# x-y20/jittor-dcn

Hardware: NVIDIA B200
Metric: DeformConv2d fwd+bwd images/sec (higher is better)
Workload: dtype f32

## Files before the change

jittor_dcn_b200/csrc/dcn_umma_bwd_data.cu:

```cuda
#include <cstdlib>
#include <cstring>
#include <type_traits>

#include "dcn_umma.h"
#include "dcn_umma_common.cuh"

namespace dcn {

using namespace ptx;

namespace bd {

constexpr int kScatWarps = 16;
constexpr int kMmaWarp = kScatWarps, kLoadWarp = kScatWarps + 1;
constexpr int kFirstPlanWarp = kScatWarps + 2;
__host__ __device__ constexpr int threads_of(int pw) { return (kFirstPlanWarp + pw) * 32; }
constexpr int kPlanPerThread = 8;
__host__ __device__ constexpr int plan_max_of(int pw) { return pw * 32 * kPlanPerThread; }
constexpr uint32_t kGImg = 128 * 64 * 2;

struct __align__(16) ScatEntry {
  uint32_t base;
  float fx, fy;
  uint32_t gidx;
};
constexpr uint32_t kDeadEntry = 0xffffffffu;

struct Params {
  Geo g;
  Tiling t;
  const void* xt;
  float* gxt;
  const float* off;
  const void* gout;
  const uint8_t* wtiles;
  const uint8_t* gtiles;
  float* gb_fused;
  int row_v;
  float* goff;
  float scale_iy, scale_ix;
  int Gt, Rt, chunks, num_inst;
  int num_tiles;
  FastDiv divR, divChunks;
  int pix_blocks;
  int ix_delta;
  int ncols;
  int cblocks;
  int OB;
  int plan_cap;
  int fuse_w;
  int o_halves;
  int o_cols;
  float* gw;
  int nslices, nchunks, cb_per_slice;
  int g_imgs;
  int g_nbuf;
  uint32_t g_img;
  uint32_t w_stage;
  uint32_t tmem_cols;
  int w_resident;
  int w_ring;
};

struct PlanWork {
  float ox, oy;
  int h, w, n, chan_base, valid;
  uint32_t gidx;
  float mk;
};

template <int VARIANT, bool PLAIN = false, bool MOD = false>
__device__ __forceinline__ void plan_prepare(const Params& P, int tile, int cb, int e, PlanWork& pw,
                                             const float* __restrict__ mask = nullptr) {
  const Geo& g = P.g;
  pw.valid = 0;
  pw.ox = pw.oy = 0.f;
  pw.h = pw.w = pw.n = pw.chan_base = 0;
  pw.gidx = kDeadEntry;
  uint32_t p, n, h, w;
  int b;
  if (VARIANT == DCN_VARIANT_TORCH) {
    const int il = e >> (P.ncols == 128 ? 7 : 6), cc = e & (P.ncols - 1), j = cb * P.ncols + cc;
    const TileRowInfo ri = decode_inst(P, tile * P.Rt + il);
    if (!ri.valid || j >= g.K) return;
    uint32_t cbase, q;
    P.t.divP.divmod((uint32_t)(ri.r0 * g.K + j), cbase, q);
    P.t.divN.divmod(q, p, n);
    pw.chan_base = (int)cbase * P.t.G + ri.chunk * P.Gt;
    b = ri.b;
  } else {
    const int tl = e >> (P.ncols == 128 ? 7 : 6), cc = e & (P.ncols - 1);
    b = tile / P.pix_blocks;
    p = (uint32_t)((tile - b * P.pix_blocks) * P.ncols + cc);
    n = P.t.divC.div((uint32_t)(cb * 128)) + (uint32_t)tl;
// ... 38 lines not shown
__device__ __forceinline__ ScatEntry plan_finish(const Geo& g, const PlanWork& pw) {
  ScatEntry e;
  int base = xt_null_base(g);
  e.fx = e.fy = 0.f;
  e.gidx = kDeadEntry;
  if (pw.valid) {
    const Tap tp = tap_of(g, pw.h, pw.w, pw.n, pw.ox, pw.oy);
    bool inside;
    base = xt_corner_base(g, tp.y0, tp.x0, inside);
    if (inside) {
      e.fx = tp.fx;
      e.fy = tp.fy;
      e.gidx = pw.gidx;
    }
  }
  e.base = 4u * (uint32_t)(base + pw.chan_base);
  return e;
}

template <int S, int NV>
__device__ __forceinline__ void reduce_scatter(float (&v)[NV], unsigned mask, int lane) {
#pragma unroll
  for (int s = S, n = NV / 2; n >= 1; s >>= 1, n >>= 1) {
    const bool up = (lane & s) != 0;
#pragma unroll
    for (int k = 0; k < n; ++k) {
      const float send = up ? v[k] : v[k + n];
      const float keep = up ? v[k + n] : v[k];
      v[k] = keep + __shfl_xor_sync(mask, send, s);
    }
  }
}

template <int VARIANT, int RW, bool FUSE, bool BF, int PW, bool PLAIN = false, bool MOD = false>
__global__ void __launch_bounds__(threads_of(PW), 1) bwd_data_kernel(const __grid_constant__ Params P,
                                                                     const float* __restrict__ mask,
                                                                     float* __restrict__ gmask) {
  constexpr int NIMG = BF ? 1 : 2;
  typedef typename std::conditional<BF, __nv_bfloat16, float>::type XT;
  extern __shared__ __align__(1024) uint8_t smem_raw[];
  uint8_t* smem = smem_raw + ((1024u - (smem_u32(smem_raw) & 1023u)) & 1023u);
  const Geo& g = P.g;
  uint8_t* gtile = smem;
  const uint32_t g_buf = (uint32_t)P.OB * NIMG * P.g_img;
  const uint32_t g_zero_off = (uint32_t)P.g_nbuf * g_buf;
  uint8_t* wstage = gtile + g_zero_off + (size_t)(P.g_imgs - P.OB) * NIMG * P.g_img;
  uint8_t* sbuf = wstage + (size_t)(P.w_resident ? P.w_resident : P.w_ring) * P.w_stage;
  const uint32_t s_img = 128u * 128u, s_buf = FUSE ? NIMG * s_img : 0u;
  ScatEntry* plan = reinterpret_cast<ScatEntry*>(sbuf + 2 * (size_t)s_buf);
  float* mplan = reinterpret_cast<float*>(plan + 2 * P.plan_cap);
  uint64_t* bars = MOD ? reinterpret_cast<uint64_t*>(mplan + 2 * P.plan_cap)
                       : reinterpret_cast<uint64_t*>(plan + 2 * P.plan_cap);
  uint64_t* wfull = bars;
  uint64_t* wempty = bars + 2;
  uint64_t* tfull = bars + 4;
  uint64_t* tempty = bars + 6;
  uint64_t* pfull = bars + 8;
  uint64_t* pempty = bars + 10;
  uint64_t* gfull = bars + 12;
  uint64_t* gempty = bars + 14;
  uint64_t* sfull = bars + 16;
  uint64_t* sempty = bars + 18;
  uint64_t* dfull = bars + 20;
  uint32_t* tmem_slot = reinterpret_cast<uint32_t*>(bars + 21);
  {
    uint32_t dyn;
    asm volatile("mov.u32 %0, %%dynamic_smem_size;" : "=r"(dyn));
    if (smem_u32(tmem_slot + 1) - smem_u32(smem_raw) > dyn) __trap();
  }

  const int tid = threadIdx.x, warp = tid >> 5, lane = tid & 31;
  const int ncols = P.ncols;

  if (tid == 0) {
    for (int a = 0; a < 2; ++a) {
      mbar_init(&wfull[a], 1);
      mbar_init(&wempty[a], 1);
      mbar_init(&tfull[a], 1);
      mbar_init(&tempty[a], kScatWarps);
      mbar_init(&pfull[a], PW);
      mbar_init(&pempty[a], kScatWarps);
    }
    for (int a = 0; a < 2; ++a) {
      mbar_init(&gfull[a], 1);
      mbar_init(&gempty[a], 1);
      mbar_init(&sfull[a], kScatWarps);
      mbar_init(&sempty[a], 1);
    }
    mbar_init(dfull, 1);
    fence_barrier_init();
  }
  if (warp == 0) {
    asm volatile("tcgen05.alloc.cta_group::1.sync.aligned.shared::cta.b32 [%0], %1;" ::"r"(
                     smem_u32(tmem_slot)),
                 "r"(P.tmem_cols)
                 : "memory");
    asm volatile("tcgen05.relinquish_alloc_permit.cta_group::1.sync.aligned;" ::: "memory");
  }
  if (FUSE) {
    const uint32_t zero_end = g_zero_off + (uint32_t)(P.g_imgs - P.OB) * NIMG * P.g_img;
    for (uint32_t i = g_zero_off + tid * 16; i < zero_end; i += threads_of(PW) * 16)
      *reinterpret_cast<uint4*>(gtile + i) = make_uint4(0, 0, 0, 0);
    fence_proxy_async_smem();
  }
  tc_fence_before();
  __syncthreads();
  tc_fence_after();
  const uint32_t tmem_base = *tmem_slot;
  const size_t img_stride = xt_image_stride(g);
  int tile0, tile_step, cb0, cb1;
  if (!FUSE) {
    tile0 = blockIdx.x;
    tile_step = gridDim.x;
    cb0 = 0;
    cb1 = P.cblocks;
  } else {
    const int slice = blockIdx.x % P.nslices;
    tile0 = blockIdx.x / P.nslices;
    tile_step = P.nchunks;
    cb0 = slice * P.cb_per_slice;
    cb1 = min(P.cblocks, cb0 + P.cb_per_slice);
  }
  const uint32_t d2_base = tmem_base + 2u * (uint32_t)P.ncols;

  if (warp < kScatWarps) {
    const int quarter = warp & 3, part = warp >> 2;
    const int m = quarter * 32 + lane;
    const int cols_per_part = ncols >> 2;
    const unsigned grp_mask = RW == 32 ? 0xffffffffu : (0xffffu << (lane & 16));
    const int gl = lane & (RW - 1);
    int acc = 0, pb = 0, sb = 0;
    uint32_t acc_phase = 0, pphase = 0, sphase = 0;
    const int dg1 = 4 * g.C, dg2 = 4 * xt_row_pitch(g);
    const int dx1 = (int)sizeof(XT) * g.C, dx2 = (int)sizeof(XT) * xt_row_pitch(g);
    for (int tile = tile0; tile < P.num_tiles; tile += tile_step) {
      int slot = 0, chan = 0, bimg = 0;
      if (VARIANT == DCN_VARIANT_TORCH) {
        slot = m / P.Gt;
        chan = m - slot * P.Gt;
        bimg = decode_inst(P, tile * P.Rt + slot).b;
      } else {
        bimg = tile / P.pix_blocks;
      }
      for (int cb = cb0; cb < cb1; ++cb) {
        int mrow = 0;
        if (VARIANT != DCN_VARIANT_TORCH) {
          const int j = cb * 128 + m, n = j / g.C;
          chan = j - n * g.C;
          slot = n - (cb * 128) / g.C;
          if (MOD) mrow = (bimg * g.N + n) * g.HW + (tile - bimg * P.pix_blocks) * ncols;
        }
        const char* ximg =
            reinterpret_cast<const char*>(reinterpret_cast<const XT*>(P.xt) + (size_t)bimg * img_stride + chan);
        char* gimg = P.gxt ? reinterpret_cast<char*>(P.gxt + (size_t)bimg * img_stride + chan) : nullptr;
        mbar_wait_relaxed(&tfull[acc], acc_phase, 32);
        mbar_wait_relaxed(&pfull[pb], pphase, 32);
// ... 275 lines not shown
            uint32_t raw[8];
            asm volatile("tcgen05.ld.sync.aligned.32x32b.x8.b32 {%0,%1,%2,%3,%4,%5,%6,%7}, [%8];"
                         : "=r"(raw[0]), "=r"(raw[1]), "=r"(raw[2]), "=r"(raw[3]), "=r"(raw[4]), "=r"(raw[5]),
                           "=r"(raw[6]), "=r"(raw[7])
                         : "r"(taddr + c0)
                         : "memory");
            asm volatile("tcgen05.wait::ld.sync.aligned;" ::: "memory");
            if (j < g.K) {
#pragma unroll
              for (int u = 0; u < 8; ++u)
                if (c0 + u < g.O) atomicAdd(P.gw + wt_index(g, c0 + u, j), __uint_as_float(raw[u]));
            }
          }
        }
      }
      tc_fence_before();
    }
  } else if (warp == kMmaWarp) {
    {
      const uint32_t idesc = make_idesc_bf16(128, ncols, false, false);
      const uint32_t idesc_w = make_idesc_bf16(128, ncols, true, true);
      int s = 0, acc = 0, sb = 0, gb = 0;
      uint32_t phase = 0, acc_phase = 0, gphase = 0, sphase = 0;
      bool first_tile = true;
      const uint32_t idesc_wj = make_idesc_bf16(128, P.o_cols > 0 ? P.o_cols : 16, false, true);
      auto wgrad_mmas = [&](int cb, bool first, int gb) {
        mbar_wait_relaxed(&sfull[sb], sphase, 32);
        tc_fence_after();
        const uint32_t g_hi = smem_u32(gtile) + (uint32_t)gb * g_buf, g_lo = g_hi + P.g_img;
        const uint32_t sbase = smem_u32(sbuf + (size_t)sb * s_buf);
        if (VARIANT == DCN_VARIANT_TORCH) {
          const uint64_t ds0 = make_sdesc_sw128(sbase, 1024, 1024);
          const uint32_t gimg16 = P.g_img >> 4;
          for (int hf = 0; hf < P.o_halves; ++hf) {
            const uint32_t g_h = g_hi + (uint32_t)(2 * hf) * NIMG * P.g_img;
            const uint32_t g_lbo = 2 * hf + 1 < P.OB ? NIMG * P.g_img
                                                     : g_zero_off - (uint32_t)gb * g_buf - (uint32_t)(2 * hf) * NIMG * P.g_img;
            const uint32_t d_tmem = d2_base + (uint32_t)((hf * P.cb_per_slice + cb - cb0) * ncols);
            const uint64_t dg0 = make_sdesc_sw128(g_h, g_lbo, 1024);
            if (elect_one()) {
#pragma unroll
              for (int ks = 0; ks < 8; ++ks) {
                const uint64_t dgh = dg0 + (uint64_t)(ks * 128), dsh = ds0 + (uint64_t)(ks * 128);
                umma_bf16(d_tmem, dgh, dsh, idesc_w, (first && ks == 0) ? 0u : 1u);
                if (!BF) {
                  umma_bf16(d_tmem, dgh, dsh + (s_img >> 4), idesc_w, 1u);
                  umma_bf16(d_tmem, dgh + gimg16, dsh, idesc_w, 1u);
                }
              }
            }
            __syncwarp();
          }
        } else {
          const uint32_t g_lbo = NIMG * P.g_img;
          const uint32_t d_tmem = d2_base + (uint32_t)((cb - cb0) * P.o_cols);
          const uint64_t ds0 = make_sdesc_sw128(sbase, 16, 1024), dg0 = make_sdesc_sw128(g_hi, g_lbo, 1024);
          const uint32_t gimg16 = P.g_img >> 4;
          if (elect_one()) {
#pragma unroll
            for (int k4 = 0; k4 < 4; ++k4) {
              const uint64_t dsh = ds0 + (uint64_t)(k4 * 2), dgh = dg0 + (uint64_t)(k4 * 128);
              umma_bf16(d_tmem, dsh, dgh, idesc_wj, (first && k4 == 0) ? 0u : 1u);
              if (!BF) {
                umma_bf16(d_tmem, dsh, dgh + gimg16, idesc_wj, 1u);
                umma_bf16(d_tmem, dsh + (s_img >> 4), dgh, idesc_wj, 1u);
              }
            }
          }
        }
        if (elect_one()) umma_commit(&sempty[sb]);
// ... 80 lines not shown
        }
        first_tile = false;
      }
      if (FUSE) drain();
      if (FUSE && elect_one()) umma_commit(dfull);
      __syncwarp();
    }
  } else if (warp == kLoadWarp) {
    if (lane == 0) {
      int s = 0;
      uint32_t phase = 0;
      if (P.w_resident) {
        if (tile0 < P.num_tiles) {
          const int n = (cb1 - cb0) * P.OB;
          mbar_arrive_expect_tx(&wfull[0], (uint32_t)n * P.w_stage);
          for (int i = 0; i < n; ++i)
            bulk_g2s(wstage + (size_t)i * P.w_stage, P.wtiles + ((size_t)cb0 * P.OB + i) * P.w_stage, P.w_stage,
                     &wfull[0]);
        }
      } else
      for (int tile = tile0; tile < P.num_tiles; tile += tile_step) {
        for (int cb = cb0; cb < cb1; ++cb)
          for (int ob = 0; ob < P.OB; ++ob) {
            mbar_wait_relaxed(&wempty[s], phase ^ 1, 32);
            mbar_arrive_expect_tx(&wfull[s], P.w_stage);
            bulk_g2s(wstage + (size_t)s * P.w_stage, P.wtiles + (size_t)(cb * P.OB + ob) * P.w_stage,
                     P.w_stage, &wfull[s]);
            if (++s == P.w_ring) {
              s = 0;
              phase ^= 1;
            }
          }
      }
    } else if (lane == 1) {
      uint32_t gphase = 0;
      int gb = 0;
      for (int tile = tile0; tile < P.num_tiles; tile += tile_step) {
        mbar_wait_relaxed(&gempty[gb], gphase ^ 1, 64);
        mbar_arrive_expect_tx(&gfull[gb], g_buf);
        if (VARIANT == DCN_VARIANT_TORCH || ncols == 128) {
          bulk_g2s(gtile + (size_t)gb * g_buf, P.gtiles + (size_t)tile * g_buf, g_buf, &gfull[gb]);
        } else {
          const int b = tile / P.pix_blocks, pblk = tile - b * P.pix_blocks;
          const int pb128 = (g.HW + 127) / 128;
          const uint8_t* src = P.gtiles + ((size_t)(b * pb128 + (pblk >> 1)) * P.OB * NIMG) * kGImg + (pblk & 1) * (kGImg / 2);
          for (int i = 0; i < P.OB * NIMG; ++i)
            bulk_g2s(gtile + (size_t)gb * g_buf + (size_t)i * P.g_img, src + (size_t)i * kGImg, P.g_img, &gfull[gb]);
        }
        if (++gb == P.g_nbuf) {
          gb = 0;
          gphase ^= 1;
        }
      }
    }
  } else {
    const int pt = tid - kFirstPlanWarp * 32;
    constexpr int kPlanThreads = PW * 32;
    const int n_ent = P.plan_cap;
    int pb = 0;
    uint32_t pphase = 0;
    PlanWork pw[kPlanPerThread];
    if (tile0 < P.num_tiles) {
#pragma unroll
      for (int u = 0; u < kPlanPerThread; ++u)
        if (pt + u * kPlanThreads < n_ent) plan_prepare<VARIANT, PLAIN, MOD>(P, tile0, cb0, pt + u * kPlanThreads, pw[u], mask);
    }
    for (int tile = tile0; tile < P.num_tiles; tile += tile_step) {
      for (int cb = cb0; cb < cb1; ++cb) {
        ScatEntry* pl = plan + pb * P.plan_cap;
        mbar_wait_relaxed(&pempty[pb], pphase ^ 1, 64);
#pragma unroll
        for (int u = 0; u < kPlanPerThread; ++u)
          if (pt + u * kPlanThreads < n_ent)
            pl[pt + u * kPlanThreads] = PLAIN ? plan_finish_plain(g, pw[u]) : plan_finish(g, pw[u]);
        if (MOD) {
          float* mpl = mplan + pb * P.plan_cap;
#pragma unroll
          for (int u = 0; u < kPlanPerThread; ++u)
            if (pt + u * kPlanThreads < n_ent) mpl[pt + u * kPlanThreads] = pw[u].valid ? pw[u].mk : 0.f;
        }
        __syncwarp();
        if (lane == 0) mbar_arrive(&pfull[pb]);
        int ntile = tile, ncb = cb + 1;
        if (ncb == cb1) {
          ncb = cb0;
// ... 121 lines not shown
    for (int q = 0; q < 8; ++q) v[q] = tile[ck * 8 + q][row];
    uint4 hi, lo;
    split_pair(v[0], v[1], hi.x, lo.x);
    split_pair(v[2], v[3], hi.y, lo.y);
    split_pair(v[4], v[5], hi.z, lo.z);
    split_pair(v[6], v[7], hi.w, lo.w);
    const uint32_t so = kmajor_sw128_off(row, ck * 8);
    *reinterpret_cast<uint4*>(img + so) = hi;
    if (NIMG == 2) *reinterpret_cast<uint4*>(img + img_bytes + so) = lo;
  }
}

template <typename T>
__global__ void __launch_bounds__(256) weight_tiles_bwd_kernel(Geo g, int ncols, int cblocks, int OB,
                                                               const T* __restrict__ wt,
                                                               uint8_t* __restrict__ tiles) {
  constexpr int NIMG = sizeof(T) == 2 ? 1 : 2;
  const int total = cblocks * ncols * OB * 64;
  const uint32_t img = (uint32_t)ncols * 128;
  for (int i = blockIdx.x * blockDim.x + threadIdx.x; i < total; i += gridDim.x * blockDim.x) {
    const int o = i % (OB * 64), jj = i / (OB * 64);
    const int cb = jj / ncols, jl = jj - cb * ncols, ob = o >> 6, ol = o & 63;
    const float v = (o < g.O && jj < g.K) ? (float)wt[wt_index(g, o, jj)] : 0.f;
    __nv_bfloat16 hi, lo;
    ptx::split_bf16(v, hi, lo);
    uint8_t* base = tiles + (size_t)(cb * OB + ob) * NIMG * img + ptx::kmajor_sw128_off(jl, ol);
    *reinterpret_cast<__nv_bfloat16*>(base) = hi;
    if (NIMG == 2) *reinterpret_cast<__nv_bfloat16*>(base + img) = lo;
  }
}

}

static void choose_slices(bd::Params* P, int max_cb, size_t real, size_t zero, size_t other) {
  const int ns_min = (P->cblocks + max_cb - 1) / max_cb;
  double best = 1e30;
  for (int ns = ns_min; ns <= ns_min + 2 && ns <= P->cblocks; ++ns) {
    const int cbp = (P->cblocks + ns - 1) / ns;
    const int ns_eff = (P->cblocks + cbp - 1) / cbp;
    const double waste = (double)ns_eff * cbp / P->cblocks * 148.0 / (ns_eff * (148 / ns_eff));
    if (waste < best - 1e-9) {
      best = waste;
      P->nslices = ns_eff;
      P->cb_per_slice = cbp;
    }
  }
  const size_t n_res = (size_t)P->cb_per_slice * P->OB;
  const int plans[5][3] = {{2, 1, 2}, {2, 0, 2}, {2, 0, 1}, {1, 1, 2}, {1, 0, 2}};
  for (const auto& pl : plans) {
    const size_t n_w = pl[1] ? n_res : (size_t)pl[2];
    const size_t need = pl[0] * real + zero + n_w * P->w_stage + other;
    if (need <= kSmemBudget || (pl[2] == 1 && need - 768 <= kSmemBudget)) {
      P->g_nbuf = pl[0];
      P->w_resident = pl[1] ? (int)n_res : 0;
      P->w_ring = pl[2];
      return;
    }
  }
}

static bool copy_row_tiling(const Geo& g, bd::Params* P) {
  if (!make_tiling(g, &P->t)) return false;
  P->Gt = P->t.Gt;
  P->Rt = P->t.Rt;
  P->chunks = P->t.chunks;
  P->num_inst = P->t.num_inst;
  P->num_tiles = P->t.num_tiles;
  P->divR = P->t.divR;
  P->divChunks = P->t.divChunks;
  return true;
}

static bool bwd_data_tiling(const Geo& g, int operand, bd::Params* P) {
  const size_t nimg = operand == DCN_OPERAND_BF16 ? 1 : 2;
  if (!copy_row_tiling(g, P)) return false;
  P->fuse_w = 0;
  P->o_halves = 1;
  P->o_cols = 0;
  P->w_resident = 0;
  P->w_ring = 2;
  P->g_nbuf = 1;
  P->gw = nullptr;
  P->nslices = P->nchunks = 1;
  P->cb_per_slice = 0;
  if ((long long)g.B * 2 * g.N * g.HW > 0xffffffffLL) return false;
  if ((long long)xt_image_stride(g) >= (1LL << 30)) return false;
  P->OB = (g.O + 63) / 64;
  if (P->OB > 4) return false;
  const bool torch = g.variant == DCN_VARIANT_TORCH;
  if (!torch && !(g.C % 128 == 0 || g.C == 64 || g.C == 32 || g.C == 16)) return false;
  const int ent = torch ? P->t.Rt : (g.C >= 128 ? 1 : 128 / g.C);
  const int halves = g.O > 128 ? 2 : 1;
  const int o_cols = (g.O + 15) / 16 * 16;
  const int max_cb = torch ? 6 / halves : min((512 - 2 * 64) / o_cols, 8);
  const size_t zero = torch ? (size_t)(2 * halves - P->OB) * nimg * bd::kGImg : 0;
  const struct { bool fuse; int ncols; } cands[3] = {{true, 64}, {false, 128}, {false, 64}};
  for (const auto& c : cands) {
    const int ncols = c.ncols;
    const int w_rows = torch ? ncols : 128;
    const uint32_t g_img = torch ? bd::kGImg : (uint32_t)ncols * 128;
    const uint32_t w_stage = (uint32_t)nimg * w_rows * 128;
    const size_t real = (size_t)P->OB * nimg * g_img, z = c.fuse ? zero : 0;
    const size_t rest = 2 * (size_t)w_stage + (c.fuse ? 2 * nimg * (size_t)(128 * 128) : 0) +
                        2 * (size_t)ent * ncols * sizeof(bd::ScatEntry) + 256 + 1024;
    if (ent * ncols > bd::plan_max_of(4) || real + z + rest > kSmemBudget) continue;
    P->ncols = ncols;
    P->cblocks = (g.K + w_rows - 1) / w_rows;
    P->plan_cap = ent * ncols;
    P->g_img = g_img;
    P->w_stage = w_stage;
    P->pix_blocks = torch ? 1 : (g.HW + ncols - 1) / ncols;
    P->num_tiles = torch ? P->t.num_tiles : g.B * P->pix_blocks;
    P->g_imgs = c.fuse && torch ? 2 * halves : P->OB;
    P->tmem_cols = c.fuse ? 512 : 2 * ncols;
    if (!c.fuse) {
      P->g_nbuf = (2 * real + rest <= kSmemBudget) ? 2 : 1;
      return true;
    }
    P->fuse_w = 1;
    if (torch) P->o_halves = halves;
    else P->o_cols = o_cols;
    choose_slices(P, max_cb, real, z, rest - 2 * (size_t)w_stage);
    return true;
  }
  return false;
}

bool umma_bwd_data_supported(const Geo& g, int operand) {
  if (operand != DCN_OPERAND_FP32 && operand != DCN_OPERAND_BF16) return false;
  bd::Params P;
  P.g = g;
  return bwd_data_tiling(g, operand, &P);
}

bool umma_bwd_data_fuses_wgrad(const Geo& g, int operand) {
  bd::Params P;
  P.g = g;
  return bwd_data_tiling(g, operand, &P) && P.fuse_w;
}

size_t umma_bwd_data_wtile_bytes(const Geo& g, int operand) {
  bd::Params P;
  P.g = g;
  if (!bwd_data_tiling(g, operand, &P)) return 0;
  return align_up((size_t)P.cblocks * P.OB * P.w_stage, 1024);
}

static int launch_gout_tiles(const bd::Params& P, bool bf, uint8_t* gtiles, cudaStream_t st) {
  const dim3 grid((unsigned)(((size_t)P.num_tiles * P.t.Rt + bd::kGtInst - 1) / bd::kGtInst),
                  (unsigned)((P.OB * 64 / bd::kGtOsub) * (P.t.Gt / bd::kGtCh)));
  KernelScope scope("gout_tiles_kernel", st);
  if (bf)
    bd::gout_tiles_torch_kernel<__nv_bfloat16><<<grid, 256, 0, st>>>(P, gtiles);
  else
    bd::gout_tiles_torch_kernel<float><<<grid, 256, 0, st>>>(P, gtiles);
// ... 8 lines not shown
int launch_gout_tiles_pix(const Geo& g, int operand, const void* gout, uint8_t* gtiles, cudaStream_t st) {
  const int OB = (g.O + 63) / 64;
  const dim3 grid((unsigned)((g.HW + 127) / 128), (unsigned)OB, (unsigned)g.B);
  KernelScope scope("gout_tiles_kernel", st);
  if (operand == DCN_OPERAND_BF16)
    bd::gout_tiles_pix_kernel<__nv_bfloat16><<<grid, 256, 0, st>>>(g, OB, (const __nv_bfloat16*)gout, gtiles);
  else
    bd::gout_tiles_pix_kernel<float><<<grid, 256, 0, st>>>(g, OB, (const float*)gout, gtiles);
  DCN_KERNEL_CHECK("gout_tiles_kernel");
  return DCN_OK;
}

size_t umma_wgrad_gtile_bytes(const Geo& g, int operand) {
  Tiling t;
  if (!make_tiling(g, &t)) return 0;
  if (g.variant != DCN_VARIANT_TORCH) return gtile_pix_bytes(g, operand);
  return align_up((size_t)t.num_tiles * ((g.O + 63) / 64) * (operand == DCN_OPERAND_BF16 ? 1 : 2) * bd::kGImg, 1024);
}
int launch_gout_tiles_fwd_order(const Geo& g, int operand, const void* gout, uint8_t* gtiles, cudaStream_t st) {
  if (g.variant != DCN_VARIANT_TORCH) return launch_gout_tiles_pix(g, operand, gout, gtiles, st);
  bd::Params P;
  memset(&P, 0, sizeof(P));
  P.g = g;
  if (!copy_row_tiling(g, &P)) return DCN_ERR_UNSUPPORTED;
  P.OB = (g.O + 63) / 64;
  P.gout = gout;
  P.row_v = operand == DCN_OPERAND_BF16 ? 8 : 4;
  return launch_gout_tiles(P, operand == DCN_OPERAND_BF16, gtiles, st);
}

size_t umma_bwd_data_gtile_bytes(const Geo& g, int operand) {
  bd::Params P;
  P.g = g;
  if (!bwd_data_tiling(g, operand, &P)) return 0;
  if (g.variant != DCN_VARIANT_TORCH) return gtile_pix_bytes(g, operand);
  return align_up((size_t)P.num_tiles * P.OB * (operand == DCN_OPERAND_BF16 ? 1 : 2) * bd::kGImg, 1024);
}

struct BdLaunch {
  const bd::Params& P;
  int grid;
  size_t smem;
  cudaStream_t st;
  const float* mask;
  float* gmask;
};

template <int VARIANT, int RW, bool FUSE, bool BF, int PW, bool PLAIN, bool MOD>
static int launch_bd(const BdLaunch& L) {
  DCN_CUDA_TRY(cudaFuncSetAttribute(bd::bwd_data_kernel<VARIANT, RW, FUSE, BF, PW, PLAIN, MOD>,
                                    cudaFuncAttributeMaxDynamicSharedMemorySize, (int)L.smem));
  bd::bwd_data_kernel<VARIANT, RW, FUSE, BF, PW, PLAIN, MOD>
      <<<L.grid, bd::threads_of(PW), L.smem, L.st>>>(L.P, L.mask, L.gmask);
  DCN_KERNEL_CHECK("umma_bwd_data_kernel");
  return DCN_OK;
}

template <int VARIANT, bool FUSE, bool BF, bool PLAIN, bool MOD>
static int launch_bd_split(const BdLaunch& L, bool narrow) {
  if (narrow) return launch_bd<VARIANT, 16, FUSE, BF, 4, PLAIN, MOD>(L);
  if (L.P.plan_cap <= 128) return launch_bd<VARIANT, 32, FUSE, BF, 2, PLAIN, MOD>(L);
  return launch_bd<VARIANT, 32, FUSE, BF, 4, PLAIN, MOD>(L);
}

template <int VARIANT, bool MOD>
static int launch_bd_operand(const BdLaunch& L, bool bf, bool narrow) {
  if (bf)
    return L.P.fuse_w ? launch_bd_split<VARIANT, true, true, false, MOD>(L, narrow)
                      : launch_bd_split<VARIANT, false, true, false, MOD>(L, narrow);
  return L.P.fuse_w ? launch_bd_split<VARIANT, true, false, false, MOD>(L, narrow)
                    : launch_bd_split<VARIANT, false, false, false, MOD>(L, narrow);
}

int umma_bwd_data_any(const Geo& g, int operand, const void* xt, float* gxt, const float* off, const void* wt,
                      const void* gout, float* goff, float* gw, uint8_t* wtiles, uint8_t* gtiles,
                      cudaStream_t st, float* gb_fused, const float* mask, float* gmask) {
  bd::Params P;
  P.g = g;
  const bool bf = operand == DCN_OPERAND_BF16;
  const size_t nimg = bf ? 1 : 2;
  if (!bwd_data_tiling(g, operand, &P)) {
    set_error("umma bwd_data: shape not tileable");
    return DCN_ERR_UNSUPPORTED;
  }
  {
    const int rows = g.variant == DCN_VARIANT_TORCH ? P.ncols : 128;
    const int total = P.cblocks * rows * P.OB * 64;
    KernelScope scope("weight_tiles_bwd_kernel", st);
    if (bf)
      bd::weight_tiles_bwd_kernel<__nv_bfloat16><<<min((total + 255) / 256, 2048), 256, 0, st>>>(
          g, rows, P.cblocks, P.OB, (const __nv_bfloat16*)wt, wtiles);
    else
      bd::weight_tiles_bwd_kernel<float><<<min((total + 255) / 256, 2048), 256, 0, st>>>(g, rows, P.cblocks, P.OB,
                                                                                       (const float*)wt, wtiles);
    DCN_KERNEL_CHECK("weight_tiles_bwd_kernel");
  }
  P.xt = xt;
  P.gxt = gxt;
  P.off = off;
  P.gout = gout;
  P.wtiles = wtiles;
  P.gtiles = gtiles;
  P.row_v = 0;
  P.gb_fused = g.variant == DCN_VARIANT_TORCH ? gb_fused : nullptr;
  {
    int rc = g.variant == DCN_VARIANT_TORCH ? launch_gout_tiles(P, bf, gtiles, st)
                                            : launch_gout_tiles_pix(g, operand, gout, gtiles, st);
    if (rc) return rc;
  }
  P.goff = goff;
  P.gw = gw;
  P.ix_delta = (off_col_ch(g, 0) - off_row_ch(g, 0)) * g.HW;
  P.scale_iy = g.variant == DCN_VARIANT_DCNV1 ? 1.f : g.sy * 2.0f / g.Dx;
  P.scale_ix = g.variant == DCN_VARIANT_DCNV1 ? 1.f : g.sx * 2.0f / g.Dy;
  size_t smem = ((size_t)P.g_nbuf * P.OB + (P.g_imgs - P.OB)) * nimg * P.g_img +
                (size_t)(P.w_resident ? P.w_resident : P.w_ring) * P.w_stage +
                (P.fuse_w ? 2 * nimg * (size_t)(128 * 128) : 0) +
                2 * (size_t)P.plan_cap * sizeof(bd::ScatEntry) + 256 + 1024;
  if (mask) smem += 2 * (size_t)P.plan_cap * sizeof(float);
  if (smem > kSmemBudget) smem = kSmemBudget;
  const int sms = num_sms();
  int grid = P.num_tiles < sms ? P.num_tiles : sms;
  if (P.fuse_w) {
    P.nchunks = sms / P.nslices;
    if (P.nchunks < 1) P.nchunks = 1;
    if (P.nchunks > P.num_tiles) P.nchunks = P.num_tiles;
    grid = P.nslices * P.nchunks;
  }
  const BdLaunch L{P, grid, smem, st, mask, gmask};
  const bool narrow = g.variant == DCN_VARIANT_TORCH ? P.t.Gt == 16 : g.C == 16;
  KernelScope scope(g.plain ? "umma_offset_conv_bwd_kernel" : "umma_bwd_data_kernel", st);
  if (g.plain) {
    if (g.variant == DCN_VARIANT_TORCH || bf || !P.fuse_w) {
      set_error("plain (offset-conv) backward: pixel-row layout, fp32 operands, fused weight gradient only");
      return DCN_ERR_UNSUPPORTED;
    }
    return launch_bd_split<DCN_VARIANT_JITTOR, true, false, true, false>(L, narrow);
  }
  if (mask) {
    if (g.variant != DCN_VARIANT_DCNV1 || !gmask) {
      set_error("umma bwd_data: a mask exists for the DCNv1 variant only, and needs grad_mask");
      return DCN_ERR_UNSUPPORTED;
    }
    return launch_bd_operand<DCN_VARIANT_JITTOR, true>(L, bf, narrow);
  }
  if (g.variant == DCN_VARIANT_TORCH) return launch_bd_operand<DCN_VARIANT_TORCH, false>(L, bf, narrow);
  return launch_bd_operand<DCN_VARIANT_JITTOR, false>(L, bf, narrow);
}

}
```

jittor_dcn_b200/csrc/dcn_umma_fwd.cu:

```cuda
#include <cuda.h>

#include <cstdlib>
#include <cstring>
#include <type_traits>

#include "dcn_umma.h"
#include "dcn_umma_common.cuh"

namespace dcn {

using namespace ptx;

constexpr int kEpiWarps = 4, kFirstPlanWarp = kEpiWarps + 2;
constexpr int kPlanMax = 512;
constexpr uint32_t kATile = 128 * 64 * 2;
constexpr uint32_t kAMnLbo = 1024, kAMnSbo = 2048;
constexpr int kMaxStages = 4;
constexpr int kFwdStages = 3;

enum { MODE_FWD = 0, MODE_WGRAD = 1 };

struct FwdParams {
  Geo g;
  Tiling t;
// ... 811 lines not shown
  if (operand == DCN_OPERAND_BF16 && g.C % 8) return false;
  Tiling t;
  return tiling_ok(g, &t);
}

static size_t elem_bytes(int operand) { return operand == DCN_OPERAND_BF16 ? 2 : 4; }

size_t umma_xt_bytes(const Geo& g, int operand) {
  return align_up(elem_bytes(operand) * (size_t)g.B * xt_image_stride(g), 1024);
}

size_t umma_fwd_workspace(const Geo& g, int operand) {
  Tiling t;
  make_tiling(g, &t);
  const int nimg = operand == DCN_OPERAND_BF16 ? 1 : 2;
  return umma_xt_bytes(g, operand) + align_up((size_t)t.KB * nimg * g.O * 128, 1024);
}

typedef CUresult (*EncodeTiledFn)(CUtensorMap*, CUtensorMapDataType, cuuint32_t, void*, const cuuint64_t*,
                                  const cuuint64_t*, const cuuint32_t*, const cuuint32_t*, CUtensorMapInterleave,
                                  CUtensorMapSwizzle, CUtensorMapL2promotion, CUtensorMapFloatOOBfill);
static EncodeTiledFn encode_tiled_fn() {
  static EncodeTiledFn fn = [] {
    void* p = nullptr;
    cudaDriverEntryPointQueryResult q;
    if (cudaGetDriverEntryPoint("cuTensorMapEncodeTiled", &p, cudaEnableDefault, &q) != cudaSuccess ||
        q != cudaDriverEntryPointSuccess)
      p = nullptr;
    return (EncodeTiledFn)p;
  }();
  return fn;
}

static bool make_out_tensor_map(const Geo& g, const Tiling& t, int box_r, float* out, CUtensorMap* map) {
  EncodeTiledFn enc = encode_tiled_fn();
  if (!enc) return false;
  const cuuint64_t dims[4] = {(cuuint64_t)t.R, (cuuint64_t)t.G, (cuuint64_t)g.O, (cuuint64_t)g.B};
  const cuuint64_t strides[3] = {(cuuint64_t)t.R * 4, (cuuint64_t)g.HW * 4, (cuuint64_t)g.Oimg * g.HW * 4};
  const cuuint32_t box[4] = {(cuuint32_t)box_r, (cuuint32_t)t.Gt, (cuuint32_t)g.O, 1};
  const cuuint32_t estr[4] = {1, 1, 1, 1};
  return enc(map, CU_TENSOR_MAP_DATA_TYPE_FLOAT32, 4, out, dims, strides, box, estr, CU_TENSOR_MAP_INTERLEAVE_NONE,
             CU_TENSOR_MAP_SWIZZLE_NONE, CU_TENSOR_MAP_L2_PROMOTION_NONE,
             CU_TENSOR_MAP_FLOAT_OOB_FILL_NONE) == CUDA_SUCCESS;
}

static void common_params(const Geo& g, FwdParams& P) {
  const int n_ent = g.variant == DCN_VARIANT_TORCH ? P.t.Rt * 64 : 128 * P.t.taps_per_kb;
  P.plan_cap = (n_ent + 255) / 256 * 256;
  P.gout = nullptr;
  P.gw = nullptr;
  P.gtiles = nullptr;
  P.g_OB = 0;
  P.nslices = P.nchunks = P.kb_per_slice = 1;
  P.o_blocks = 1;
  P.n_gbuf = 0;
  P.g_img = 0;
  P.tma_out = 0;
  P.tpg = 1;
  P.n_ost = 1;
  P.box_r = 0;
  P.stage_out_bytes = 0;
  P.kperm_slabs = 0;
  P.mask = nullptr;
}

template <int VARIANT, int MODE, bool BF, bool PLAIN, int PW, int GW, bool MOD>
static int launch_umma_gemm(const FwdParams& P, const CUtensorMap& tmap, int grid, size_t smem, cudaStream_t st) {
  DCN_CUDA_TRY(cudaFuncSetAttribute(umma_gemm_kernel<VARIANT, MODE, BF, PLAIN, PW, GW, MOD>,
                                    cudaFuncAttributeMaxDynamicSharedMemorySize, (int)smem));
  umma_gemm_kernel<VARIANT, MODE, BF, PLAIN, PW, GW, MOD>
      <<<grid, (kFirstPlanWarp + PW + GW) * 32, smem, st>>>(P, tmap);
  DCN_KERNEL_CHECK(MODE == MODE_FWD ? "umma_fwd_kernel" : "umma_bwd_weight_kernel");
  return DCN_OK;
}
// ... 35 lines not shown
}

int umma_forward_any(const Geo& g, int operand, const void* x, const float* off, const void* wt,
                     const float* bias, float* out, void* workspace, cudaStream_t st, bool stage_x,
                     const float* mask) {
  FwdParams P;
  P.g = g;
  if (!make_tiling(g, &P.t)) {
    set_error("umma forward: shape not tileable");
    return DCN_ERR_UNSUPPORTED;
  }
  common_params(g, P);
  const int nimg = operand == DCN_OPERAND_BF16 ? 1 : 2;
  void* xt = workspace;
  uint8_t* wtiles = (uint8_t*)workspace + umma_xt_bytes(g, operand);
  int rc;
  if (stage_x && (rc = launch_nchw_to_nhwc(g, P.t, x, xt, operand, st))) return rc;
  if ((rc = launch_weight_tiles_fwd(g, P.t, wt, wtiles, operand, st))) return rc;
  P.xt = xt;
  P.off = off;
  P.wtiles = wtiles;
  P.bias = bias;
  P.out = out;
  P.mask = mask;
  P.b_tile = (uint32_t)g.O * 128;
  P.stage_bytes = nimg * (kATile + P.b_tile);
  size_t fixed = 2 * (size_t)P.plan_cap * sizeof(PlanEntry) + 256 + 1024;
  alignas(64) CUtensorMap tmap;
  memset(&tmap, 0, sizeof(tmap));
  if (g.variant == DCN_VARIANT_TORCH && P.t.Rt == 2 && !g.out_framed) {
    const int box_r = P.t.Rt < 4 ? 4 : P.t.Rt;
    const size_t bytes = sizeof(float) * (size_t)g.O * P.t.Gt * box_r;
    if (P.t.R % box_r == 0 && bytes <= 64 * 1024 && g.O <= 256 &&
        (size_t)2 * P.stage_bytes + bytes + fixed <= kSmemBudget && make_out_tensor_map(g, P.t, box_r, out, &tmap)) {
      P.tma_out = 1;
      P.box_r = box_r;
      P.tpg = box_r / P.t.Rt;
      P.stage_out_bytes = (uint32_t)align_up(bytes, 1024);
      P.n_ost = (size_t)3 * P.stage_bytes + 2 * P.stage_out_bytes + fixed <= kSmemBudget ? 2 : 1;
      fixed += (size_t)P.n_ost * P.stage_out_bytes;
    }
  }
  const int stages = (int)((kSmemBudget - fixed) / P.stage_bytes);
  P.stages = stages > kFwdStages ? kFwdStages : stages;
  if (P.stages < 2) {
    set_error("umma forward: not enough shared memory for 2 stages");
    return DCN_ERR_UNSUPPORTED;
  }
  P.tmem_cols = pow2_cols(2 * g.O);
  if (g.variant != DCN_VARIANT_TORCH && g.C % 64 == 0 && g.C > 64 && P.t.KB == g.N * (g.C / 64))
    P.kperm_slabs = g.C / 64;
  const size_t smem = (size_t)P.stages * P.stage_bytes + fixed;
  const int sms = num_sms();
  const int groups = (P.t.num_tiles + P.tpg - 1) / P.tpg;
  const int grid = groups < sms ? groups : sms;
  KernelScope scope(g.plain ? "umma_offset_conv_fwd_kernel" : "umma_fwd_kernel", st);
  return launch_gemm<MODE_FWD>(g, operand, P, tmap, grid, smem, st);
}

bool conv_offset_fwd_supported(const Geo& g, int O);
size_t conv_offset_wtile_bytes(const Geo& g, int O);
int conv_offset_forward(const Geo& g, const float* xt, const float* woff, const float* boff, float* offset_out,
                        uint8_t* wtiles, cudaStream_t st, float* mask_out);

bool umma_offset_conv_fwd_supported(const Geo& g, int n_out) {
  Tiling t;
  if (!make_tiling(g, &t)) return false;
// ... 92 lines not shown
```

Before: 18560.

## Fuse grad_out staging into bwd-data kernel via TMA loads and in-kernel bf16 split

```diff
diff --git a/jittor_dcn_b200/csrc/dcn_umma_bwd_data.cu b/jittor_dcn_b200/csrc/dcn_umma_bwd_data.cu
--- a/jittor_dcn_b200/csrc/dcn_umma_bwd_data.cu
+++ b/jittor_dcn_b200/csrc/dcn_umma_bwd_data.cu
@@ -1,3 +1,5 @@
+#include <cuda.h>
+
 #include <cstdlib>
 #include <cstring>
 #include <type_traits>
@@ -53,13 +55,14 @@
   int o_cols;
   float* gw;
   int nslices, nchunks, cb_per_slice;
-  int g_imgs;
   int g_nbuf;
   uint32_t g_img;
   uint32_t w_stage;
   uint32_t tmem_cols;
   int w_resident;
   int w_ring;
+  int gin;
+  uint32_t raw_bytes;
 };
 
 struct PlanWork {
@@ -164,19 +167,53 @@
   }
 }
 
+__device__ __forceinline__ void convert_box(const float4* __restrict__ raw, uint8_t* img, uint32_t g_img, int rsub,
+                                            int chunk0, int i, int lane, float* bias) {
+  const bool upper = rsub != 0;
+#pragma unroll
+  for (int ck = 0; ck < 2; ++ck) {
+    float pb[8];
+    uint32_t hw[2][4], lw[2][4];
+#pragma unroll
+    for (int u = 0; u < 8; u += 2) {
+      const float4 a = raw[(ck * 8 + u) * 64 + i], b = raw[(ck * 8 + u + 1) * 64 + i];
+      const float a0 = upper ? a.z : a.x, a1 = upper ? a.w : a.y;
+      const float b0 = upper ? b.z : b.x, b1 = upper ? b.w : b.y;
+      split_pair(a0, b0, hw[0][u >> 1], lw[0][u >> 1]);
+      split_pair(a1, b1, hw[1][u >> 1], lw[1][u >> 1]);
+      pb[u] = a0 + a1;
+      pb[u + 1] = b0 + b1;
+    }
+#pragma unroll
+    for (int h = 0; h < 2; ++h) {
+      uint8_t* dst = img + kmajor_sw128_off(h * 64 + i, (chunk0 + ck) * 8);
+      *reinterpret_cast<uint4*>(dst) = make_uint4(hw[h][0], hw[h][1], hw[h][2], hw[h][3]);
+      *reinterpret_cast<uint4*>(dst + g_img) = make_uint4(lw[h][0], lw[h][1], lw[h][2], lw[h][3]);
+    }
+    if (bias) {
+      reduce_scatter<16>(pb, 0xffffffffu, lane);
+      pb[0] += __shfl_xor_sync(0xffffffffu, pb[0], 2);
+      pb[0] += __shfl_xor_sync(0xffffffffu, pb[0], 1);
+      if ((lane & 3) == 0) bias[ck * 8 + (lane >> 2)] += pb[0];
+    }
+  }
+}
+
 template <int VARIANT, int RW, bool FUSE, bool BF, int PW, bool PLAIN = false, bool MOD = false>
 __global__ void __launch_bounds__(threads_of(PW), 1) bwd_data_kernel(const __grid_constant__ Params P,
                                                                      const float* __restrict__ mask,
-                                                                     float* __restrict__ gmask) {
+                                                                     float* __restrict__ gmask,
+                                                                     const __grid_constant__ CUtensorMap tmap_gout) {
   constexpr int NIMG = BF ? 1 : 2;
+  constexpr bool CONVERT = VARIANT == DCN_VARIANT_TORCH && RW == 32 && FUSE && !BF && PW == 2 && !PLAIN && !MOD;
   typedef typename std::conditional<BF, __nv_bfloat16, float>::type XT;
   extern __shared__ __align__(1024) uint8_t smem_raw[];
   uint8_t* smem = smem_raw + ((1024u - (smem_u32(smem_raw) & 1023u)) & 1023u);
   const Geo& g = P.g;
   uint8_t* gtile = smem;
   const uint32_t g_buf = (uint32_t)P.OB * NIMG * P.g_img;
-  const uint32_t g_zero_off = (uint32_t)P.g_nbuf * g_buf;
-  uint8_t* wstage = gtile + g_zero_off + (size_t)(P.g_imgs - P.OB) * NIMG * P.g_img;
+  uint8_t* graw = gtile + (size_t)P.g_nbuf * g_buf;
+  uint8_t* wstage = graw + P.raw_bytes;
   uint8_t* sbuf = wstage + (size_t)(P.w_resident ? P.w_resident : P.w_ring) * P.w_stage;
   const uint32_t s_img = 128u * 128u, s_buf = FUSE ? NIMG * s_img : 0u;
   ScatEntry* plan = reinterpret_cast<ScatEntry*>(sbuf + 2 * (size_t)s_buf);
@@ -194,7 +231,8 @@
   uint64_t* sfull = bars + 16;
   uint64_t* sempty = bars + 18;
   uint64_t* dfull = bars + 20;
-  uint32_t* tmem_slot = reinterpret_cast<uint32_t*>(bars + 21);
+  uint64_t* rfull = bars + 21;
+  uint32_t* tmem_slot = reinterpret_cast<uint32_t*>(bars + 23);
   {
     uint32_t dyn;
     asm volatile("mov.u32 %0, %%dynamic_smem_size;" : "=r"(dyn));
@@ -220,6 +258,8 @@
       mbar_init(&sempty[a], 1);
     }
     mbar_init(dfull, 1);
+    mbar_init(&rfull[0], 1);
+    mbar_init(&rfull[1], 1);
     fence_barrier_init();
   }
   if (warp == 0) {
@@ -228,12 +268,6 @@
                  "r"(P.tmem_cols)
                  : "memory");
     asm volatile("tcgen05.relinquish_alloc_permit.cta_group::1.sync.aligned;" ::: "memory");
-  }
-  if (FUSE) {
-    const uint32_t zero_end = g_zero_off + (uint32_t)(P.g_imgs - P.OB) * NIMG * P.g_img;
-    for (uint32_t i = g_zero_off + tid * 16; i < zero_end; i += threads_of(PW) * 16)
-      *reinterpret_cast<uint4*>(gtile + i) = make_uint4(0, 0, 0, 0);
-    fence_proxy_async_smem();
   }
   tc_fence_before();
   __syncthreads();
@@ -254,6 +288,62 @@
     cb1 = min(P.cblocks, cb0 + P.cb_per_slice);
   }
   const uint32_t d2_base = tmem_base + 2u * (uint32_t)P.ncols;
+
+  auto convert_gout = [&]() {
+    const uint32_t box = (P.raw_bytes - 1024u) / 2u;
+    const int nq = 4 * P.OB;
+    float* sbias = P.gb_fused != nullptr && blockIdx.x % P.nslices == 0
+                       ? reinterpret_cast<float*>(graw + 2 * box) : nullptr;
+    if (sbias)
+      for (int o = lane; o < 256; o += 32) sbias[o] = 0.f;
+    auto issue = [&](int tile, int q, int slot) {
+      const TileRowInfo ri = decode_inst(P, tile * P.Rt);
+      mbar_arrive_expect_tx(&rfull[slot], box);
+      asm volatile(
+          "cp.async.bulk.tensor.4d.shared::cluster.global.mbarrier::complete_tx::bytes [%0], [%1, {%3, %4, %5, %6}], "
+          "[%2];" ::"r"(smem_u32(graw + slot * box)),
+          "l"(reinterpret_cast<uint64_t>(&tmap_gout)), "r"(smem_u32(&rfull[slot])), "r"(ri.r0 & ~3), "r"(ri.chunk * P.Gt),
+          "r"(16 * q), "r"(ri.b)
+          : "memory");
+    };
+    int it = tile0, iq = 0;
+    auto issue_next = [&](int slot) {
+      if (it >= P.num_tiles) return;
+      if (lane == 0) issue(it, iq, slot);
+      if (++iq == nq) {
+        iq = 0;
+        it += tile_step;
+      }
+    };
+    issue_next(0);
+    issue_next(1);
+    uint32_t gphase = 0;
+    int gb = 0, k = 0;
+    for (int tile = tile0; tile < P.num_tiles; tile += tile_step) {
+      const int rsub = decode_inst(P, tile * P.Rt).r0 & 3;
+      uint8_t* gdst = gtile + (size_t)gb * g_buf;
+      mbar_wait_relaxed(&gempty[gb], gphase ^ 1, 64);
+      for (int q = 0; q < nq; ++q, ++k) {
+        const int slot = k & 1;
+        mbar_wait_relaxed(&rfull[slot], (uint32_t)(k >> 1) & 1u, 32);
+        for (int i = lane; i < 64; i += 32)
+          convert_box(reinterpret_cast<const float4*>(graw + slot * box), gdst + (size_t)(q >> 2) * NIMG * P.g_img,
+                      P.g_img, rsub, 2 * (q & 3), i, lane, sbias ? sbias + 16 * q : nullptr);
+        if (q == nq - 1) fence_proxy_async_smem();
+        __syncwarp();
+        if (q == nq - 1 && lane == 0) mbar_arrive(&gfull[gb]);
+        issue_next(slot);
+      }
+      if (++gb == P.g_nbuf) {
+        gb = 0;
+        gphase ^= 1;
+      }
+    }
+    if (sbias) {
+      __syncwarp();
+      for (int o = lane; o < g.O; o += 32) atomicAdd(P.gb_fused + o, sbias[o]);
+    }
+  };
 
   if (warp < kScatWarps) {
     const int quarter = warp & 3, part = warp >> 2;
@@ -595,10 +685,9 @@
         if (VARIANT == DCN_VARIANT_TORCH) {
           const uint64_t ds0 = make_sdesc_sw128(sbase, 1024, 1024);
           const uint32_t gimg16 = P.g_img >> 4;
+          const uint32_t g_lbo = NIMG * P.g_img;
           for (int hf = 0; hf < P.o_halves; ++hf) {
             const uint32_t g_h = g_hi + (uint32_t)(2 * hf) * NIMG * P.g_img;
-            const uint32_t g_lbo = 2 * hf + 1 < P.OB ? NIMG * P.g_img
-                                                     : g_zero_off - (uint32_t)gb * g_buf - (uint32_t)(2 * hf) * NIMG * P.g_img;
             const uint32_t d_tmem = d2_base + (uint32_t)((hf * P.cb_per_slice + cb - cb0) * ncols);
             const uint64_t dg0 = make_sdesc_sw128(g_h, g_lbo, 1024);
             if (elect_one()) {
@@ -745,7 +834,7 @@
             }
           }
       }
-    } else if (lane == 1) {
+    } else if (lane == 1 && !(CONVERT && P.gin)) {
       uint32_t gphase = 0;
       int gb = 0;
       for (int tile = tile0; tile < P.num_tiles; tile += tile_step) {
@@ -764,6 +853,12 @@
           gb = 0;
           gphase ^= 1;
         }
+      }
+    }
+    if constexpr (CONVERT) {
+      if (P.gin) {
+        __syncwarp();
+        convert_gout();
       }
     }
   } else {
@@ -951,7 +1046,23 @@
 
 }
 
-static void choose_slices(bd::Params* P, int max_cb, size_t real, size_t zero, size_t other) {
+static bool plan_smem(bd::Params* P, size_t real, size_t other) {
+  const size_t n_res = (size_t)P->cb_per_slice * P->OB;
+  const int plans[5][3] = {{2, 1, 2}, {2, 0, 2}, {2, 0, 1}, {1, 1, 2}, {1, 0, 2}};
+  for (const auto& pl : plans) {
+    const size_t n_w = pl[1] ? n_res : (size_t)pl[2];
+    const size_t need = pl[0] * real + n_w * P->w_stage + other;
+    if (need <= kSmemBudget || (pl[2] == 1 && need - 768 <= kSmemBudget)) {
+      P->g_nbuf = pl[0];
+      P->w_resident = pl[1] ? (int)n_res : 0;
+      P->w_ring = pl[2];
+      return true;
+    }
+  }
+  return false;
+}
+
+static void choose_slices(bd::Params* P, int max_cb, size_t real, size_t other, uint32_t raw) {
   const int ns_min = (P->cblocks + max_cb - 1) / max_cb;
   double best = 1e30;
   for (int ns = ns_min; ns <= ns_min + 2 && ns <= P->cblocks; ++ns) {
@@ -964,18 +1075,12 @@
       P->cb_per_slice = cbp;
     }
   }
-  const size_t n_res = (size_t)P->cb_per_slice * P->OB;
-  const int plans[5][3] = {{2, 1, 2}, {2, 0, 2}, {2, 0, 1}, {1, 1, 2}, {1, 0, 2}};
-  for (const auto& pl : plans) {
-    const size_t n_w = pl[1] ? n_res : (size_t)pl[2];
-    const size_t need = pl[0] * real + zero + n_w * P->w_stage + other;
-    if (need <= kSmemBudget || (pl[2] == 1 && need - 768 <= kSmemBudget)) {
-      P->g_nbuf = pl[0];
-      P->w_resident = pl[1] ? (int)n_res : 0;
-      P->w_ring = pl[2];
-      return;
-    }
-  }
+  if (raw && plan_smem(P, real, other + raw) && P->g_nbuf == 2 && P->w_resident) {
+    P->gin = 1;
+    P->raw_bytes = raw;
+    return;
+  }
+  plan_smem(P, real, other);
 }
 
 static bool copy_row_tiling(const Geo& g, bd::Params* P) {
@@ -1002,6 +1107,8 @@
   P->gw = nullptr;
   P->nslices = P->nchunks = 1;
   P->cb_per_slice = 0;
+  P->gin = 0;
+  P->raw_bytes = 0;
   if ((long long)g.B * 2 * g.N * g.HW > 0xffffffffLL) return false;
   if ((long long)xt_image_stride(g) >= (1LL << 30)) return false;
   P->OB = (g.O + 63) / 64;
@@ -1012,17 +1119,17 @@
   const int halves = g.O > 128 ? 2 : 1;
   const int o_cols = (g.O + 15) / 16 * 16;
   const int max_cb = torch ? 6 / halves : min((512 - 2 * 64) / o_cols, 8);
-  const size_t zero = torch ? (size_t)(2 * halves - P->OB) * nimg * bd::kGImg : 0;
+  const uint32_t raw = torch && nimg == 2 && P->t.Gt == 64 && P->t.R % 4 == 0 ? 2u * 4 * 64 * 16 * 4 + 1024u : 0u;
   const struct { bool fuse; int ncols; } cands[3] = {{true, 64}, {false, 128}, {false, 64}};
   for (const auto& c : cands) {
     const int ncols = c.ncols;
     const int w_rows = torch ? ncols : 128;
     const uint32_t g_img = torch ? bd::kGImg : (uint32_t)ncols * 128;
     const uint32_t w_stage = (uint32_t)nimg * w_rows * 128;
-    const size_t real = (size_t)P->OB * nimg * g_img, z = c.fuse ? zero : 0;
+    const size_t real = (size_t)P->OB * nimg * g_img;
     const size_t rest = 2 * (size_t)w_stage + (c.fuse ? 2 * nimg * (size_t)(128 * 128) : 0) +
                         2 * (size_t)ent * ncols * sizeof(bd::ScatEntry) + 256 + 1024;
-    if (ent * ncols > bd::plan_max_of(4) || real + z + rest > kSmemBudget) continue;
+    if (ent * ncols > bd::plan_max_of(4) || real + rest > kSmemBudget) continue;
     P->ncols = ncols;
     P->cblocks = (g.K + w_rows - 1) / w_rows;
     P->plan_cap = ent * ncols;
@@ -1030,7 +1137,6 @@
     P->w_stage = w_stage;
     P->pix_blocks = torch ? 1 : (g.HW + ncols - 1) / ncols;
     P->num_tiles = torch ? P->t.num_tiles : g.B * P->pix_blocks;
-    P->g_imgs = c.fuse && torch ? 2 * halves : P->OB;
     P->tmem_cols = c.fuse ? 512 : 2 * ncols;
     if (!c.fuse) {
       P->g_nbuf = (2 * real + rest <= kSmemBudget) ? 2 : 1;
@@ -1039,7 +1145,7 @@
     P->fuse_w = 1;
     if (torch) P->o_halves = halves;
     else P->o_cols = o_cols;
-    choose_slices(P, max_cb, real, z, rest - 2 * (size_t)w_stage);
+    choose_slices(P, max_cb, real, rest - 2 * (size_t)w_stage, raw);
     return true;
   }
   return false;
@@ -1114,9 +1220,24 @@
 size_t umma_bwd_data_gtile_bytes(const Geo& g, int operand) {
   bd::Params P;
   P.g = g;
-  if (!bwd_data_tiling(g, operand, &P)) return 0;
+  if (!bwd_data_tiling(g, operand, &P) || P.gin) return 0;
   if (g.variant != DCN_VARIANT_TORCH) return gtile_pix_bytes(g, operand);
   return align_up((size_t)P.num_tiles * P.OB * (operand == DCN_OPERAND_BF16 ? 1 : 2) * bd::kGImg, 1024);
+}
+
+bool make_out_tensor_map(const Geo& g, const Tiling& t, int box_r, int box_o, const void* ptr, CUtensorMap* map);
+
+static int stage_gout(const bd::Params& P, int operand, uint8_t* gtiles, CUtensorMap* tmap_gout, cudaStream_t st) {
+  memset(tmap_gout, 0, sizeof(*tmap_gout));
+  if (P.gin) {
+    if (!make_out_tensor_map(P.g, P.t, 4, 16, P.gout, tmap_gout)) {
+      set_error("umma bwd_data: no tensor map of grad_out (it must be 16-byte aligned)");
+      return DCN_ERR_UNSUPPORTED;
+    }
+    return DCN_OK;
+  }
+  if (P.g.variant == DCN_VARIANT_TORCH) return launch_gout_tiles(P, operand == DCN_OPERAND_BF16, gtiles, st);
+  return launch_gout_tiles_pix(P.g, operand, P.gout, gtiles, st);
 }
 
 struct BdLaunch {
@@ -1126,6 +1247,7 @@
   cudaStream_t st;
   const float* mask;
   float* gmask;
+  const CUtensorMap& tmap_gout;
 };
 
 template <int VARIANT, int RW, bool FUSE, bool BF, int PW, bool PLAIN, bool MOD>
@@ -1133,7 +1255,7 @@
   DCN_CUDA_TRY(cudaFuncSetAttribute(bd::bwd_data_kernel<VARIANT, RW, FUSE, BF, PW, PLAIN, MOD>,
                                     cudaFuncAttributeMaxDynamicSharedMemorySize, (int)L.smem));
   bd::bwd_data_kernel<VARIANT, RW, FUSE, BF, PW, PLAIN, MOD>
-      <<<L.grid, bd::threads_of(PW), L.smem, L.st>>>(L.P, L.mask, L.gmask);
+      <<<L.grid, bd::threads_of(PW), L.smem, L.st>>>(L.P, L.mask, L.gmask, L.tmap_gout);
   DCN_KERNEL_CHECK("umma_bwd_data_kernel");
   return DCN_OK;
 }
@@ -1185,9 +1307,9 @@
   P.gtiles = gtiles;
   P.row_v = 0;
   P.gb_fused = g.variant == DCN_VARIANT_TORCH ? gb_fused : nullptr;
+  alignas(64) CUtensorMap tmap_gout;
   {
-    int rc = g.variant == DCN_VARIANT_TORCH ? launch_gout_tiles(P, bf, gtiles, st)
-                                            : launch_gout_tiles_pix(g, operand, gout, gtiles, st);
+    const int rc = stage_gout(P, operand, gtiles, &tmap_gout, st);
     if (rc) return rc;
   }
   P.goff = goff;
@@ -1195,7 +1317,7 @@
   P.ix_delta = (off_col_ch(g, 0) - off_row_ch(g, 0)) * g.HW;
   P.scale_iy = g.variant == DCN_VARIANT_DCNV1 ? 1.f : g.sy * 2.0f / g.Dx;
   P.scale_ix = g.variant == DCN_VARIANT_DCNV1 ? 1.f : g.sx * 2.0f / g.Dy;
-  size_t smem = ((size_t)P.g_nbuf * P.OB + (P.g_imgs - P.OB)) * nimg * P.g_img +
+  size_t smem = (size_t)P.g_nbuf * P.OB * nimg * P.g_img + P.raw_bytes +
                 (size_t)(P.w_resident ? P.w_resident : P.w_ring) * P.w_stage +
                 (P.fuse_w ? 2 * nimg * (size_t)(128 * 128) : 0) +
                 2 * (size_t)P.plan_cap * sizeof(bd::ScatEntry) + 256 + 1024;
@@ -1209,7 +1331,7 @@
     if (P.nchunks > P.num_tiles) P.nchunks = P.num_tiles;
     grid = P.nslices * P.nchunks;
   }
-  const BdLaunch L{P, grid, smem, st, mask, gmask};
+  const BdLaunch L{P, grid, smem, st, mask, gmask, tmap_gout};
   const bool narrow = g.variant == DCN_VARIANT_TORCH ? P.t.Gt == 16 : g.C == 16;
   KernelScope scope(g.plain ? "umma_offset_conv_bwd_kernel" : "umma_bwd_data_kernel", st);
   if (g.plain) {
diff --git a/jittor_dcn_b200/csrc/dcn_umma_fwd.cu b/jittor_dcn_b200/csrc/dcn_umma_fwd.cu
--- a/jittor_dcn_b200/csrc/dcn_umma_fwd.cu
+++ b/jittor_dcn_b200/csrc/dcn_umma_fwd.cu
@@ -867,14 +867,15 @@
   return fn;
 }
 
-static bool make_out_tensor_map(const Geo& g, const Tiling& t, int box_r, float* out, CUtensorMap* map) {
+bool make_out_tensor_map(const Geo& g, const Tiling& t, int box_r, int box_o, const void* ptr, CUtensorMap* map) {
   EncodeTiledFn enc = encode_tiled_fn();
   if (!enc) return false;
   const cuuint64_t dims[4] = {(cuuint64_t)t.R, (cuuint64_t)t.G, (cuuint64_t)g.O, (cuuint64_t)g.B};
   const cuuint64_t strides[3] = {(cuuint64_t)t.R * 4, (cuuint64_t)g.HW * 4, (cuuint64_t)g.Oimg * g.HW * 4};
-  const cuuint32_t box[4] = {(cuuint32_t)box_r, (cuuint32_t)t.Gt, (cuuint32_t)g.O, 1};
+  const cuuint32_t box[4] = {(cuuint32_t)box_r, (cuuint32_t)t.Gt, (cuuint32_t)box_o, 1};
   const cuuint32_t estr[4] = {1, 1, 1, 1};
-  return enc(map, CU_TENSOR_MAP_DATA_TYPE_FLOAT32, 4, out, dims, strides, box, estr, CU_TENSOR_MAP_INTERLEAVE_NONE,
+  return enc(map, CU_TENSOR_MAP_DATA_TYPE_FLOAT32, 4, const_cast<void*>(ptr), dims, strides, box, estr,
+             CU_TENSOR_MAP_INTERLEAVE_NONE,
              CU_TENSOR_MAP_SWIZZLE_NONE, CU_TENSOR_MAP_L2_PROMOTION_NONE,
              CU_TENSOR_MAP_FLOAT_OOB_FILL_NONE) == CUDA_SUCCESS;
 }
@@ -976,7 +977,7 @@
     const int box_r = P.t.Rt < 4 ? 4 : P.t.Rt;
     const size_t bytes = sizeof(float) * (size_t)g.O * P.t.Gt * box_r;
     if (P.t.R % box_r == 0 && bytes <= 64 * 1024 && g.O <= 256 &&
-        (size_t)2 * P.stage_bytes + bytes + fixed <= kSmemBudget && make_out_tensor_map(g, P.t, box_r, out, &tmap)) {
+        (size_t)2 * P.stage_bytes + bytes + fixed <= kSmemBudget && make_out_tensor_map(g, P.t, box_r, g.O, out, &tmap)) {
       P.tma_out = 1;
       P.box_r = box_r;
       P.tpg = box_r / P.t.Rt;
```

Result: slower. 17670, median of 6 (-4.8%).
